# roahmlab/armour

Hardware: AMD Instinct MI355X
Metric: planning iters/s (eval_g+jac) Kinova 7-DOF, 100 timesteps × 20 obstacles (higher is better)
Workload: dtype f64

## Files before the change

armour_amd/csrc/api.hip:

```cpp
#include <algorithm>
#include <cmath>
#include <cstdarg>
#include <chrono>
#include <cstring>
#include <mutex>
#include <new>

#include "../../include/armour_robot_fetch.h"
#include "../../include/armour_robot_kinova.h"
#include "bezier.h"
#include "cacc.h"
#include "common.h"
#include "solver_common.h"

static thread_local char g_err[512] = "";

void armour_set_error(const char* fmt, ...) {
    va_list ap;
    va_start(ap, fmt);
    vsnprintf(g_err, sizeof(g_err), fmt, ap);
    va_end(ap);
}

extern "C" const char* armour_last_error(void) { return g_err; }
// ... 237 lines not shown
    h->d_jac = h->d_g + (size_t)B * h->m;
    const size_t bn = (size_t)B * h->n;
    h->h_q0.assign(q0, q0 + bn); h->h_qd0.assign(qd0, qd0 + bn);
    h->h_qdes.assign(q_des, q_des + bn);
    if (mode == ARMOUR_MODE_ARMTD) { h->h_qdd0.assign(bn, 0.0); h->h_krange.assign(qdd0, qdd0 + bn); }
    else { h->h_qdd0.assign(qdd0, qdd0 + bn); h->h_krange.clear(); }
    std::vector<double> bz((size_t)B * 3 * h->n);
    const double D = mode == ARMOUR_MODE_ARMTD ? 1.0 : h->params.duration;
    for (int b = 0; b < B; b++)
        for (int i = 0; i < h->n; i++) {
            bz[((size_t)b * 3 + 0) * h->n + i] = q0[b * h->n + i];
            bz[((size_t)b * 3 + 1) * h->n + i] = qd0[b * h->n + i] * D;
            bz[((size_t)b * 3 + 2) * h->n + i] = qdd0[b * h->n + i] * D * D;
        }
    HIPCHK(hipMemcpy(h->d_bez, bz.data(), bz.size() * sizeof(double), hipMemcpyHostToDevice));
    return ARMOUR_OK;
}

int armour_refresh_table_stats(ArmourPlanner* h) {
    if (h->stats_fresh) { h->stats_fresh = false; return ARMOUR_OK; }
    const size_t nl = (size_t)h->B * h->J * h->T, nt = (size_t)h->B * h->n * h->T;
    std::vector<int> lc(nl), tc(nt);
    HIPCHK(hipMemcpy(lc.data(), h->d_link_count, nl * sizeof(int), hipMemcpyDeviceToHost));
    HIPCHK(hipMemcpy(tc.data(), h->d_tq_count, nt * sizeof(int), hipMemcpyDeviceToHost));
    long long sl = 0, st = 0;
    int ml = 0, mt = 0;
    for (int v : lc) { sl += v; if (v > ml) ml = v; }
    for (int v : tc) { st += v; if (v > mt) mt = v; }
    h->sum_link = sl; h->sum_torque = st; h->max_link = ml; h->max_torque = mt;
    h->h_plane_skip.assign((size_t)h->B, 0ull);
// ... 221 lines not shown
    if (n < 1 || !q0 || !qd0 || !qdd0 || !k_range || !k || !(duration > 0)) { armour_set_error("bad argument"); return ARMOUR_EINVAL; }
    const double D = duration, s = t / D;
    for (int i = 0; i < n; i++) {
        const double a = qd0[i] * D, b = qdd0[i] * D * D, ka = k_range[i] * k[i];
        if (q) q[i] = bez::q_des(q0[i], a, b, ka, s);
        if (qd) qd[i] = bez::qd_des(q0[i], a, b, ka, s) / D;
        if (qdd) qdd[i] = bez::qdd_des(q0[i], a, b, ka, s) / (D * D);
    }
    return ARMOUR_OK;
}

extern "C" int armour_eval_g_jac_device(ArmourPlanner* h, const double* d_k, double* d_g, double* d_jac, void* stream) {
    NEED_READY(h);
    if (!d_k) { armour_set_error("d_k is null"); return ARMOUR_EINVAL; }
    const P2Tables tb = armour_make_tables(h);
    return armour_p2_launch(tb, h->max_link, h->max_torque, h->h_plane_skip.data(), d_k, d_g, d_jac, stream ? (hipStream_t)stream : h->stream);
}

static int enqueue_steps(ArmourPlanner* h, const double* d_k, int steps, double* d_g, double* d_jac, hipStream_t st) {
    const P2Tables tb = armour_make_tables(h);
    const size_t stride = (size_t)h->B * h->n;
    for (int s = 0; s < steps; s++) {
        int rc = armour_p2_launch(tb, h->max_link, h->max_torque, h->h_plane_skip.data(), d_k + (size_t)s * stride, d_g, d_jac, st);
        if (rc != ARMOUR_OK) return rc;
    }
    return ARMOUR_OK;
}

static int steps_graph(ArmourPlanner* h, const double* d_k, int steps, double* d_g, double* d_jac, hipGraphExec_t* out) {
    h->graph_clock++;
    for (auto& g : h->step_graphs)
        if (g.d_k == d_k && g.steps == steps && g.d_g == d_g && g.d_jac == d_jac) { g.last_use = h->graph_clock; *out = g.exec; return ARMOUR_OK; }
    HIPCHK(hipSetDevice(h->device));
    HIPCHK(hipStreamSynchronize(h->stream));
    hipGraph_t graph = nullptr;
    HIPCHK(hipStreamBeginCapture(h->stream, hipStreamCaptureModeThreadLocal));
    const int rc = enqueue_steps(h, d_k, steps, d_g, d_jac, h->stream);
    const hipError_t e = hipStreamEndCapture(h->stream, &graph);
// ... 38 lines not shown
            if (g.d_k == d_k && g.steps == steps && g.d_g == d_g && g.d_jac == d_jac) {
                g.last_use = ++h->graph_clock;
                HIPCHK(hipGraphLaunch(g.exec, st));
                return ARMOUR_OK;
            }
    return enqueue_steps(h, d_k, steps, d_g, d_jac, st);
}

extern "C" int armour_eval_g_jac_device_multi(ArmourPlanner* h, const double* d_k, int32_t points, double* d_g, double* d_jac,
                                              void* stream) {
    NEED_READY(h);
    if (!d_k || points < 0) { armour_set_error("bad argument"); return ARMOUR_EINVAL; }
    if (points == 0) return ARMOUR_OK;
    const P2Tables tb = armour_make_tables(h);
    const long long bn = (long long)h->B * h->n, bm = (long long)h->B * h->m;
    return armour_p2_launch(tb, h->max_link, h->max_torque, h->h_plane_skip.data(), d_k, d_g, d_jac, stream ? (hipStream_t)stream : h->stream,
                            points, bn, bm, bm * h->n);
}

int armour_spin_on_stream(hipStream_t st) {
    for (;;) {
        const hipError_t q = hipStreamQuery(st);
        if (q == hipSuccess) return ARMOUR_OK;
        if (q != hipErrorNotReady) { armour_set_error("hipStreamQuery failed: %s", hipGetErrorString(q)); return ARMOUR_EDEVICE; }
    }
}

extern "C" int armour_eval_g_jac(ArmourPlanner* h, const double* k, double* g, double* jac) {
    NEED_READY(h);
    if (!k) { armour_set_error("k is null"); return ARMOUR_EINVAL; }
    HIPCHK(hipSetDevice(h->device));
    const size_t bn = (size_t)h->B * h->n, bm = (size_t)h->B * h->m;
    const P2Tables tb = armour_make_tables(h);
    const int pinned_mode = h->tune(ARMOUR_OPT_PINNED_MODE);
    const bool all_pinned = in_pinned(k, bn * sizeof(double)) && in_pinned(g, bm * sizeof(double)) && in_pinned(jac, bm * h->n * sizeof(double));
    if (all_pinned && pinned_mode == 1) {
        int rc = armour_p2_launch(tb, h->max_link, h->max_torque, h->h_plane_skip.data(), k, g, jac, h->stream);
        if (rc != ARMOUR_OK) return rc;
        return armour_spin_on_stream(h->stream);
    }
    const double* k_dev = h->d_k;
    if (all_pinned && pinned_mode == 2) k_dev = k;
    else HIPCHK(hipMemcpyAsync(h->d_k, k, bn * sizeof(double), hipMemcpyHostToDevice, h->stream));
    int rc = armour_p2_launch(tb, h->max_link, h->max_torque, h->h_plane_skip.data(), k_dev, g ? h->d_g : nullptr, jac ? h->d_jac : nullptr, h->stream);
    if (rc != ARMOUR_OK) return rc;
    if (g && jac && jac == g + bm) {
        HIPCHK(hipMemcpyAsync(g, h->d_g, bm * (1 + (size_t)h->n) * sizeof(double), hipMemcpyDeviceToHost, h->stream));
        return armour_spin_on_stream(h->stream);
    }
    if (g) HIPCHK(hipMemcpyAsync(g, h->d_g, bm * sizeof(double), hipMemcpyDeviceToHost, h->stream));
    if (jac) HIPCHK(hipMemcpyAsync(jac, h->d_jac, bm * h->n * sizeof(double), hipMemcpyDeviceToHost, h->stream));
    return armour_spin_on_stream(h->stream);
}

extern "C" int armour_check_feasible(ArmourPlanner* h, const double* g, int32_t* feasible) {
    NEED_READY(h);
    const slv::RowRule R = armour_row_rule(h);
    const slv::RowLimits L = armour_row_limits(h);
    for (int b = 0; b < h->B; b++) {
// ... 116 lines not shown
    for (int r = tid; r < m; r += 256) p[0].take(a.rule, r, g[r], lo[r], hi[r]);
    slv::ViolPartial::tree_reduce(sh, p, tid);
    if (tid == 0) a.out[b] = slv::ViolPartial::finish(sh, 0);
}
}

static int eval_violations_device_impl(ArmourPlanner* h, const double* d_k, ArmourViolation* d_out, void* stream, bool allow_cull) {
    NEED_READY(h);
    if (!d_k || !d_out) { armour_set_error("null argument"); return ARMOUR_EINVAL; }
    HIPCHK(hipSetDevice(h->device));
    int rc = armour_upload_bounds(h);
    if (rc != ARMOUR_OK) return rc;
    const hipStream_t st = stream ? (hipStream_t)stream : h->stream;
    if (allow_cull && h->tune(ARMOUR_OPT_CULL_ROWS)) return armour_eval_violations_culled(h, d_k, d_out, st);
    const P2Tables tb = armour_make_tables(h);
    rc = armour_p2_launch(tb, h->max_link, h->max_torque, h->h_plane_skip.data(), d_k, h->d_g, nullptr, st);
    if (rc != ARMOUR_OK) return rc;
    ViolArgs a;
    a.rule = armour_row_rule(h);
    a.g = h->d_g; a.lo = h->d_bounds; a.hi = h->d_bounds + (size_t)h->B * h->m; a.out = d_out;
    hipLaunchKernelGGL(armour_violation_kernel, dim3(h->B), dim3(256), 0, st, a);
    HIPCHK(hipGetLastError());
    return ARMOUR_OK;
}

extern "C" int armour_eval_violations_device(ArmourPlanner* h, const double* d_k, ArmourViolation* d_out, void* stream) {
    return eval_violations_device_impl(h, d_k, d_out, stream, true);
}

extern "C" int armour_eval_violations(ArmourPlanner* h, const double* k, ArmourViolation* out) {
    NEED_READY(h);
// ... 174 lines not shown
```

armour_amd/csrc/common.h:

```cpp
#pragma once

#include <hip/hip_runtime.h>

#include <cstdint>
#include <cstdio>
#include <string>
#include <vector>

#include "../../include/armour_hip.h"
#include "device_mem.h"
#include "row_rules.h"

#define ARMOUR_NPLANES 36
#define ARMOUR_PLANE_COMPONENTS 5

#define ARMOUR_FIRST_LL_PLANE 21
#define ARMOUR_N_LL_PLANES 15
__host__ __device__ inline int armour_row_stride(int Q) { return (Q + 15) & ~15; }
__host__ __device__ inline size_t armour_planes_ab_offset(int Q) { (void)Q; return 0; }
__host__ __device__ inline size_t armour_planes_cd_offset(int Q) { return (size_t)2 * ARMOUR_NPLANES * armour_row_stride(Q); }
__host__ __device__ inline size_t armour_planes_dll_offset(int Q) { return (size_t)4 * ARMOUR_NPLANES * armour_row_stride(Q); }
__host__ __device__ inline size_t armour_planes_d_offset(int Q) { return (size_t)(4 * ARMOUR_NPLANES + 16) * armour_row_stride(Q); }
__host__ __device__ inline size_t armour_planes_per_problem(int Q) { return (size_t)(5 * ARMOUR_NPLANES + 16) * armour_row_stride(Q); }
__host__ __device__ inline size_t armour_plane_index(int Q, int q, int p, int c) {
// ... 87 lines not shown
    double tune_f(int option) const { return tuning[option - ARMOUR_OPT_FIRST_TUNING]; }
    DevBuf<ArmourViolation> d_viol;
    RelLists rel, rel2;
    int rel2_tq_cap = 0;
    DevBuf<unsigned char> d_sweep;
    SolveDeviceWork solve_dev;
    DevBuf<double> d_bounds;
    bool bounds_on_device = false, bounds_on_host = false;
    bool tables_from_host = false;
    std::vector<double> h_gl, h_gu;
    std::vector<double> h_q0, h_qd0, h_qdd0, h_qdes;
    std::vector<double> h_torque_radius;
    DevBuf<double> d_tr_stage;
    std::vector<double> h_link_gens;
    std::vector<unsigned long long> h_plane_skip;
    std::vector<double> h_prune_margin;
    int allocB = 0, allocO = 0;
    DevBuf<int> d_link_count;
    DevBuf<double> d_link_center;
    DevBuf<double> d_link_indep;
    DevBuf<uint32_t> d_link_keys;
    DevBuf<double> d_link_coeff;
    DevBuf<int> d_tq_count;
    DevBuf<double> d_tq_center;
    DevBuf<double> d_tq_indep;
    DevBuf<uint32_t> d_tq_keys;
    DevBuf<double> d_tq_coeff;
    DevBuf<double> d_planes;
    DevBuf<double> d_obs_center;
    int d_from_center = 0;
// ... 12 lines not shown
    bool p1_two_cu_off = false;
    int p1_hint_B = 0, p1_hint_T = 0, p1_hint_O = 0, p1_hint_builds = 0;
    int build_info[4] = {0, 0, 0, 0};
    int max_link = 0, max_torque = 0;
    long long sum_link = 0, sum_torque = 0;
    void* p1 = nullptr;
    struct StepsGraph { const double* d_k; int steps; double* d_g; double* d_jac; hipGraphExec_t exec; unsigned long long last_use; };
    std::vector<StepsGraph> step_graphs;
    unsigned long long graph_clock = 0;
};

void armour_tuning_defaults(double* tuning);
bool armour_trace_p1();
bool armour_trace_solve();

int armour_p2_launch(const P2Tables& tb, int max_link, int max_torque, const unsigned long long* h_skip, const double* d_k, double* d_g, double* d_jac, hipStream_t stream,
                     int steps = 1, long long k_stride = 0, long long g_stride = 0, long long j_stride = 0, bool skip_collision_blocks = false);
int armour_relevance_build(ArmourPlanner* h, bool for_solver);
int armour_eval_violations_culled(ArmourPlanner* h, const double* d_k, ArmourViolation* d_out, hipStream_t st);
int armour_refresh_table_stats(ArmourPlanner* h);
int armour_checked_collision_rows(const ArmourPlanner* h);
slv::RowRule armour_row_rule(const ArmourPlanner* h);
slv::RowLimits armour_row_limits(const ArmourPlanner* h);
#define NEED_READY(h)                                                                        \
    if (!(h)) { armour_set_error("null handle"); return ARMOUR_EINVAL; }                     \
    if (!(h)->ready) { armour_set_error("no problem set: call armour_set_problems first"); return ARMOUR_ESTATE; }
void armour_plan_coeffs(const ArmourPlanner* h, size_t ix, double c[3]);
double* armour_handle_pinned(ArmourPlanner* h, int slot, size_t bytes);
int armour_p2_slice_links_launch(const P2Tables& tb, const double* d_k, double* d_centers, hipStream_t stream);
P2Tables armour_make_tables(const ArmourPlanner* h);
int armour_upload_bounds(ArmourPlanner* h);
// ... 17 lines not shown
```

armour_amd/csrc/p2_eval.hip:

```cpp
#include "p2_tiles.h"

using namespace p2;

namespace {

template <bool WANT_G, bool WANT_J, bool MULTI, bool DFC, bool LL, int PPW, bool EX>
__global__ __launch_bounds__(P2_BLOCK) __attribute__((amdgpu_waves_per_eu(P2_WPE(DFC, MULTI)))) void armour_p2_eval_kernel(P2Tables tb, const double* __restrict__ k_all,
                                                                  double* __restrict__ g_all, double* __restrict__ jac_all,
                                                                  P2Launch lp) {
    extern __shared__ __attribute__((aligned(16))) unsigned char smem_raw[];
    const int b = blockIdx.y, role = blockIdx.x + lp.role0;
    const int n = tb.n, m = tb.m;
    const double* k0 = k_all + (size_t)b * n;
    double* g0 = WANT_G ? g_all + (size_t)b * m : nullptr;
    double* jac0 = WANT_J ? jac_all + (size_t)b * m * n : nullptr;
    const double k_first = ((int)threadIdx.x < n) ? k0[threadIdx.x] : 0.0;
#ifdef P2_ABLATE
    if ((P2_ABLATE & 1) && role < lp.nbc) return;
    if ((P2_ABLATE & 2) && role >= lp.nbc && role < lp.nbc + lp.nbt) return;
    if ((P2_ABLATE & 4) && role >= lp.nbc + lp.nbt) return;
#endif
    if (role < lp.nbc) collision_block<WANT_G, WANT_J, MULTI, DFC, LL, PPW, EX>(tb, lp, b, role, k0, k_first, g0, jac0, smem_raw);
    else if (role < lp.nbc + lp.nbt) torque_block<WANT_G, WANT_J, MULTI, DFC, LL, PPW, EX>(tb, lp, b, role, k0, k_first, g0, jac0, smem_raw);
    else limit_block<WANT_G, WANT_J, MULTI, DFC, LL, PPW, EX>(tb, lp, b, role, k0, k_first, g0, jac0, smem_raw);
// ... 23 lines not shown

bool armour_p2_ex_layout_ok(unsigned long long skip) {
    unsigned long long live = ~skip & ((1ull << ARMOUR_NPLANES) - 1ull);
    if (__builtin_popcountll(live) != 24) return false;
    int pl[24];
    for (int i = 0; i < 24; i++) { pl[i] = __builtin_ctzll(live); live &= live - 1ull; }
    if (pl[11] >= ARMOUR_FIRST_LL_PLANE || pl[12] < ARMOUR_FIRST_LL_PLANE) return false;
    for (int w = 2; w < 4; w++) {
        const int p0 = pl[6 * w];
        if ((p0 - ARMOUR_FIRST_LL_PLANE) & 1) return false;
        for (int i = 1; i < 6; i++) if (pl[6 * w + i] != p0 + i) return false;
    }
    return true;
}

int armour_p2_plan(const P2Tables& tb, int max_link, int max_torque, const unsigned long long* h_skip, int steps, long long k_stride,
                   long long g_stride, long long j_stride, P2Launch* lp_out, size_t* smem_out, bool* dfc_out, bool* six_out, bool* exact_out) {
    P2Launch lp;
    lp.role0 = 0;
    lp.nbc = (tb.Q + P2_ROWS - 1) / P2_ROWS;
    lp.nbt = tb.row0 == 0 ? 0 : (tb.n * tb.T + P2_TQ_ROWS - 1) / P2_TQ_ROWS;
    lp.max_pairs = tb.O > 0 ? (P2_ROWS - 1) / tb.O + 2 : 1;
    lp.strideL = max_link > 0 ? max_link : 1;
    lp.strideT = max_torque > 0 ? max_torque : 1;
    lp.skip_by_value = (tb.B == 1 && h_skip) ? 1 : 0;
    lp.skip0 = lp.skip_by_value ? h_skip[0] : 0ull;
    lp.steps = steps; lp.k_stride = k_stride; lp.g_stride = g_stride; lp.j_stride = j_stride;
    lp.magic_O = div_magic(tb.O > 0 ? tb.O : 1); lp.magic_pp3 = div_magic(3 * lp.strideL);
    if (tb.Q >= (1 << 20)) { armour_set_error("more than 2^20 collision rows per problem"); return ARMOUR_ECAPACITY; }
    if (lp.strideL * 3 > P2_BLOCK * P2_TASK_ROUNDS) { armour_set_error("link PZ with %d monomials exceeds the P2 kernel's %d", lp.strideL, P2_BLOCK * P2_TASK_ROUNDS / 3); return ARMOUR_ECAPACITY; }
    lp.pair_chunk = std::max(1, std::min(std::min(lp.max_pairs, P2_BLOCK / P2_SL), (P2_BLOCK * P2_TASK_ROUNDS) / (lp.strideL * 3)));
    if (lp.strideT > 32 * P2_TQ_ROUNDS) { armour_set_error("torque PZ with %d monomials exceeds the P2 kernel's %d", lp.strideT, 32 * P2_TQ_ROUNDS); return ARMOUR_ECAPACITY; }
    const size_t col = ((size_t)lp.max_pairs * P2_SL + (size_t)lp.pair_chunk * lp.strideL * P2_SL + 4 * 64 * 4 + 64 * ARMOUR_MAX_FACTORS) * sizeof(double) + 4 * 64 * sizeof(int);
    const size_t tq = (size_t)P2_TQ_ROWS * lp.strideT * P2_TQW * sizeof(double);
    const size_t lim = (size_t)2 * ARMOUR_MAX_FACTORS * 8 * sizeof(double);
    const size_t smem = 2 * sizeof(KPow) + std::max(std::max(col, tq), lim);
    if (smem > 64 * 1024) { armour_set_error("P2 kernel needs %zu B of LDS (link/torque monomial counts too large)", smem); return ARMOUR_ECAPACITY; }
    const bool dfc = tb.obs_center != nullptr && tb.ll_shared;
    bool six = h_skip != nullptr;
    for (int b = 0; six && b < tb.B; b++) six = __builtin_popcountll(~h_skip[b] & ((1ull << ARMOUR_NPLANES) - 1ull)) <= 24;
    bool exact = six && tb.ex_allowed && lp.max_pairs <= lp.pair_chunk;
    for (int b = 0; exact && b < tb.B; b++) exact = armour_p2_ex_layout_ok(h_skip[b]);
    *lp_out = lp; *smem_out = smem; *dfc_out = dfc; *six_out = six; *exact_out = exact;
    return ARMOUR_OK;
}

int armour_p2_launch(const P2Tables& tb, int max_link, int max_torque, const unsigned long long* h_skip, const double* d_k, double* d_g, double* d_jac,
                     hipStream_t stream, int steps, long long k_stride, long long g_stride, long long j_stride, bool skip_collision_blocks) {
    if (!d_g && !d_jac) return ARMOUR_OK;
    P2Launch lp;
    size_t smem = 0;
    bool dfc, six, exact;
    const int rc = armour_p2_plan(tb, max_link, max_torque, h_skip, steps, k_stride, g_stride, j_stride, &lp, &smem, &dfc, &six, &exact);
    if (rc != ARMOUR_OK) return rc;
    if (skip_collision_blocks) lp.role0 = lp.nbc;
    dim3 grid(lp.nbc + lp.nbt + 1 - lp.role0, tb.B), block(P2_BLOCK);
#define P2_LAUNCH_M(G, J, M)                                                                                                                      \
    do {                                                                                                                                          \
        if (dfc && exact && !(M)) hipLaunchKernelGGL((armour_p2_eval_kernel<G, J, false, true, true, 6, true>), grid, block, smem, stream, tb, d_k, d_g, d_jac, lp);      \
        else if (dfc && six) hipLaunchKernelGGL((armour_p2_eval_kernel<G, J, M, true, true, 6, false>), grid, block, smem, stream, tb, d_k, d_g, d_jac, lp);                \
        else if (dfc) hipLaunchKernelGGL((armour_p2_eval_kernel<G, J, M, true, true, 9, false>), grid, block, smem, stream, tb, d_k, d_g, d_jac, lp);              \
        else if (tb.ll_shared && exact && !(M)) hipLaunchKernelGGL((armour_p2_eval_kernel<G, J, false, false, true, 6, true>), grid, block, smem, stream, tb, d_k, d_g, d_jac, lp); \
        else if (tb.ll_shared && six) hipLaunchKernelGGL((armour_p2_eval_kernel<G, J, M, false, true, 6, false>), grid, block, smem, stream, tb, d_k, d_g, d_jac, lp); \
        else if (tb.ll_shared) hipLaunchKernelGGL((armour_p2_eval_kernel<G, J, M, false, true, 9, false>), grid, block, smem, stream, tb, d_k, d_g, d_jac, lp); \
        else hipLaunchKernelGGL((armour_p2_eval_kernel<G, J, M, false, false, 9, false>), grid, block, smem, stream, tb, d_k, d_g, d_jac, lp);             \
    } while (0)
#define P2_LAUNCH(G, J)                                                                                                     \
    do {                                                                                                                    \
// ... 19 lines not shown
```

armour_amd/csrc/p2_tiles.h:

```cpp
#pragma once
#include <algorithm>
#include <cstdlib>

#include "bezier.h"
#include "cacc.h"
#include "common.h"

#define P2_BLOCK 256
#define P2_ROWS 64
#define P2_PPW 9
#define P2_TASK_ROUNDS 2
#define P2_TQ_ROWS 8
#define P2_TQ_ROUNDS 4
#define P2_SL (3 * (1 + ARMOUR_MAX_FACTORS))
#define P2_TQW (1 + ARMOUR_MAX_FACTORS)

#define P2_WPE(DFC, MULTI) ((DFC) && !(MULTI) ? 3 : 1)

namespace p2 {


#ifdef P2_TIMELINE
#define P2_STAMP(i) do { unsigned long long t__; asm volatile("s_memrealtime %0\n\ts_waitcnt lgkmcnt(0)" : "=s"(t__) :: "memory"); stamp[i] = t__; } while (0)
#else
// ... 83 lines not shown

typedef double v2d __attribute__((ext_vector_type(2)));

struct P2Launch {
    int nbc, nbt;
    int role0;
    int max_pairs;
    int strideL;
    int strideT;
    int pair_chunk;
    int skip_by_value;
    unsigned long long skip0;
    int steps;
    long long k_stride, g_stride, j_stride;
    unsigned long long magic_O, magic_pp3;
};

struct PassRegs {
    uint32_t tkey[P2_TASK_ROUNDS];
    double tco[P2_TASK_ROUNDS];
    int tcnt[P2_TASK_ROUNDS], tdst[P2_TASK_ROUNDS];
    double rc_cen, rc_ind;
    int rc_cnt;
};

__device__ inline void load_pass(const P2Tables& tb, const P2Launch& lp, int b, int lt_first, int p0, int pc, PassRegs& pr) {
    const int tid = threadIdx.x;
    const int per_pair = lp.strideL * P2_SL, per_pair3 = lp.strideL * 3;
    const int ntask = pc * per_pair3;
#pragma unroll
// ... 73 lines not shown
    int* pneg = reinterpret_cast<int*>(part + 4 * 64 * 4);
    double* stage = part + 4 * 64 * 4 + 4 * 64 / 2;

    const int q_begin = role * P2_ROWS;
    const int q_end = min(Q, q_begin + P2_ROWS);
    const int q = min(q_begin + lane, q_end - 1);
    const size_t Qs = (size_t)armour_row_stride(Q);
    const double* pl0 = tb.planes + (size_t)b * armour_planes_per_problem(Q);
    const v2d* plAB = reinterpret_cast<const v2d*>(pl0) + q;
    const v2d* plCD = reinterpret_cast<const v2d*>(pl0 + armour_planes_cd_offset(Q)) + q;
    const v2d* plLL = reinterpret_cast<const v2d*>(pl0 + armour_planes_dll_offset(Q)) + q;
    const double* plD = pl0 + armour_planes_d_offset(Q) + q;
    const int JT = tb.J * T;
    const int q_lt = fast_div(q, lp.magic_O), q_o = q - q_lt * O;
    const double* pll = tb.planes_ll + (size_t)b * armour_planes_ll_per_problem(JT) + (size_t)q_lt * ARMOUR_LL_RECORD;
    unsigned long long live = ~(lp.skip_by_value ? lp.skip0 : tb.plane_skip[b]) & ((1ull << ARMOUR_NPLANES) - 1ull);
    const bool plane0_live = (live & 1ull) != 0;
    const int na = __popcll(live), base = na >> 2, rem = na & 3;
    const int my_cnt = base + (wv < rem ? 1 : 0), my_start = wv * base + min(wv, rem);
    for (int s = 0; s < my_start; s++) live &= live - 1ull;
    double a0[PPW], a1[PPW], a2[PPW], dd[PPW], dl[PPW];
    const int lt_first = q_begin / O;
    const int npairs = (q_end - 1) / O - lt_first + 1;
    const bool single_pass = npairs <= lp.pair_chunk;
    PassRegs pr;
    if (EX) load_pass_uncond(tb, lp, b, lt_first, npairs, pr);
    v2d raw[EX ? 12 : 1];
    bool ll_wave = false;
    if (EX) {
        static_assert(!EX || PPW == 6, "the EX kernels hold six planes per wave");
        ll_wave = wv >= 2;
        const v2d* ra[12];
        const double* da[6];
        if (ll_wave) {
            const int pll0 = __builtin_ctzll(live) - ARMOUR_FIRST_LL_PLANE;
            const v2d* nrm = reinterpret_cast<const v2d*>(pll + (size_t)pll0 * 3);
#pragma unroll
            for (int j = 0; j < 9; j++) ra[j] = nrm + j;
// ... 261 lines not shown
}

template <bool WANT_G, bool WANT_J, bool MULTI, bool DFC, bool LL, int PPW, bool EX>
__device__ __forceinline__ void limit_block(const P2Tables& tb, const P2Launch& lp, const int b, const int role, const double* __restrict__ k0,
                                   const double k_first, double* __restrict__ g0_in, double* __restrict__ jac0_in, unsigned char* smem_raw) {
    KPow* kp2 = reinterpret_cast<KPow*>(smem_raw);
    double* lds = reinterpret_cast<double*>(smem_raw + 2 * sizeof(KPow));
    const int n = tb.n, T = tb.T, O = tb.O, Q = tb.Q, m = tb.m;
    const int tid = threadIdx.x, lane = tid & 63;
    const int wv = __builtin_amdgcn_readfirstlane(tid >> 6);
    double* g0 = WANT_G ? g0_in : nullptr;
    double* jac0 = WANT_J ? jac0_in : nullptr;
    const int nsteps = MULTI ? lp.steps : 1;
    double k_next = k_first;
    (void)lane; (void)wv; (void)T; (void)O; (void)Q; (void)m; (void)kp2; (void)lds; (void)g0; (void)jac0; (void)nsteps; (void)k_next;
    double* pv = lds;
    const int jv = tid >> 3, piece = tid & 7;
    const double* bz = tb.bez + (size_t)b * 3 * n;
    if (tb.mode == ARMOUR_MODE_ARMTD) {
        for (int s = 0; s < nsteps; s++) {
            const double* k = k0 + (size_t)s * lp.k_stride;
            double* g = WANT_G ? g0 + (size_t)s * lp.g_stride : nullptr;
            double* jac = WANT_J ? jac0 + (size_t)s * lp.j_stride : nullptr;
            if (tid < n) {
                const cacc::Extrema e = cacc::joint_extrema(bz[tid], bz[n + tid], bz[2 * n + tid] * k[tid]);
                const cacc::Cand c4[4] = {e.q_min, e.q_max, e.qd_min, e.qd_max};
                const size_t off = (size_t)tb.row0 + Q;
                for (int r = 0; r < 4; r++) {
                    const size_t row = off + (size_t)r * n + tid;
                    if (WANT_G) g[row] = c4[r].v;
                    if (WANT_J) for (int c = 0; c < n; c++) jac[row * n + c] = (c == tid) ? c4[r].d : 0.0;
                }
            }
        }
        return;
    }
    for (int s = 0; s < nsteps; s++) {
        const double* k = k0 + (size_t)s * lp.k_stride;
        double* g = WANT_G ? g0 + (size_t)s * lp.g_stride : nullptr;
        double* jac = WANT_J ? jac0 + (size_t)s * lp.j_stride : nullptr;
        if (jv < 2 * n && piece < 6) {
            const int i = jv % n;
            const bool vel = jv >= n;
            const double q0 = bz[i], a = bz[n + i], bb = bz[2 * n + i], ka = tb.k_range[i] * k[i];
            double e2, e3, v;
            if (!vel) bez::q_stationary(a, bb, ka, &e2, &e3); else bez::qd_stationary(a, bb, ka, &e2, &e3);
            if (piece < 4) {
                const double tt = piece == 0 ? 0.0 : piece == 1 ? e2 : piece == 2 ? e3 : 1.0;
                v = vel ? bez::qd_des(q0, a, bb, ka, tt) : bez::q_des(q0, a, bb, ka, tt);
            } else {
                const int sg = piece == 4 ? +1 : -1;
                v = vel ? bez::qd_extremum_dk(q0, a, bb, ka, sg) : bez::q_extremum_dk(q0, a, bb, ka, sg);
            }
            pv[jv * 8 + piece] = v;
            if (piece == 1) pv[jv * 8 + 6] = e2;
            if (piece == 2) pv[jv * 8 + 7] = e3;
        }
        __syncthreads();
        if (tid < 2 * n) {
            const int i = tid % n;
            const bool vel = tid >= n;
            const double* v = pv + tid * 8;
            const double v1 = v[0], v2 = v[1], v3 = v[2], v4 = v[3], e2 = v[6], e3 = v[7];
            double mn, mx;
            int mnId, mxId;
            if (v1 < v4) { mn = v1; mnId = 1; mx = v4; mxId = 4; } else { mn = v4; mnId = 4; mx = v1; mxId = 1; }
            if (0 <= e2 && e2 <= 1) { if (v2 < mn) { mn = v2; mnId = 2; } if (mx < v2) { mx = v2; mxId = 2; } }
            if (0 <= e3 && e3 <= 1) { if (v3 < mn) { mn = v3; mnId = 3; } if (mx < v3) { mx = v3; mxId = 3; } }
            const double sc = vel ? tb.k_range[i] / tb.duration : tb.k_range[i];
            const double dmn = (mnId == 1 ? 0.0 : mnId == 2 ? v[4] : mnId == 3 ? v[5] : 1.0) * sc;
            const double dmx = (mxId == 1 ? 0.0 : mxId == 2 ? v[4] : mxId == 3 ? v[5] : 1.0) * sc;
            const size_t off = (size_t)tb.row0 + Q;
            const size_t r_mn = off + (vel ? 2 * n : 0) + i, r_mx = r_mn + n;
            if (WANT_G) { g[r_mn] = vel ? mn / tb.duration : mn; g[r_mx] = vel ? mx / tb.duration : mx; }
            if (WANT_J) {
                for (int c = 0; c < n; c++) {
                    jac[r_mn * n + c] = (c == i) ? dmn : 0.0;
                    jac[r_mx * n + c] = (c == i) ? dmx : 0.0;
                }
            }
        }
        __syncthreads();
    }
}

}
```

armour_amd/csrc/relevance.hip:

```cpp
#include <vector>

#include "p2_sparse.h"

using namespace p2;

namespace {

constexpr double kRelMargin = 1e-9;

struct RelTables {
    P2Tables tb;
    const double* lo; const double* hi;
    unsigned char* rel;
    unsigned char* rel2;
    int* tq_tiles; int* tq_count; int tq_cap;
    int* rows; int* count;
    int* rows_res; int* count_res;
    double* packed; const long long* pack_off;
};

__device__ inline PlaneVals load_plane(const P2Tables& tb, const double* pl0, const double* pll, int Q, int q, int p, bool dfc, double oc0, double oc1, double oc2) {
    PlaneVals v;
    if (tb.ll_shared && p >= ARMOUR_FIRST_LL_PLANE) {
        const double* al = pll + (size_t)(p - ARMOUR_FIRST_LL_PLANE) * 3;
// ... 353 lines not shown
        if (aux_count) HIPCHK(hipMemcpy(aux_count, L.count + B, B * sizeof(int), hipMemcpyDeviceToHost));
    }
    if (pack_off) {
        std::vector<long long> d_off(2 * B);
        HIPCHK(hipMemcpy(d_off.data(), L.pack_off, 2 * B * sizeof(long long), hipMemcpyDeviceToHost));
        for (size_t i = 0; i < 2 * B; i++) pack_off[i] = d_off[i];
    }
    if (packed && total > 0) HIPCHK(hipMemcpy(packed, L.packed, (size_t)total * sizeof(double), hipMemcpyDeviceToHost));
    return ARMOUR_OK;
}

int armour_eval_violations_culled(ArmourPlanner* h, const double* d_k, ArmourViolation* d_out, hipStream_t st) {
    int rc = armour_relevance_build(h, false);
    if (rc != ARMOUR_OK) return rc;
    const P2Tables tb = armour_make_tables(h);
    rc = armour_p2_launch(tb, h->max_link, h->max_torque, h->h_plane_skip.data(), d_k, h->d_g, nullptr, st, 1, 0, 0, 0, true);
    if (rc != ARMOUR_OK) return rc;
    RelTables a;
    a.tb = tb;
    a.lo = h->d_bounds; a.hi = h->d_bounds + (size_t)h->B * h->m;
    a.rel = h->rel.mask; a.rows = h->rel.rows; a.count = h->rel.count; a.rows_res = h->rel.extra; a.count_res = h->rel.count + (size_t)h->B;
    a.packed = h->rel.packed; a.pack_off = h->rel.pack_off;
    if (h->rel.max_count > 0)
        hipLaunchKernelGGL(armour_sparse_collision_g_kernel, dim3((h->rel.max_count + 63) / 64, h->B), dim3(64), 0, st, a, d_k, h->d_g);
    SparseViolArgs v;
    v.rule = armour_row_rule(h);
    v.g = h->d_g; v.lo = a.lo; v.hi = a.hi; v.rows_res = a.rows_res; v.count_res = a.count_res; v.k = d_k; v.out = d_out;
    hipLaunchKernelGGL(armour_sparse_violation_kernel, dim3(h->B), dim3(256), 0, st, v);
    HIPCHK(hipGetLastError());
    return ARMOUR_OK;
}
// ... 1 lines not shown
```

armour_amd/csrc/solver_device.h:

```cpp
#pragma once
#include "common.h"
#include "p2_tiles.h"
#include "p2_sparse.h"
#include "solver_common.h"

struct alignas(128) SolveCtl {
    unsigned go;
    int pad0;
    double x[slv::NV];
};
struct alignas(64) BlockWord {
    unsigned flag;
    int count;
    int bad;
    int pad0;
    long long viol;
};

struct SolveArgs {
    P2Tables tb;
    p2::P2Launch lp;
    int nb, n_tiles;
    int culled;
    p2::SparseList sl;
// ... 17 lines not shown
    long long budget_ticks;
    long long hard_ticks;
    long long* stamps;
};

struct SolvePlan {
    p2::P2Launch lp;
    size_t smem;
    bool six;
    int n_tiles;
    int capacity;
    double ticks_per_ms;
    const void* fn;
};

int armour_p2_plan(const P2Tables& tb, int max_link, int max_torque, const unsigned long long* h_skip, int steps, long long k_stride,
                   long long g_stride, long long j_stride, p2::P2Launch* lp_out, size_t* smem_out, bool* dfc_out, bool* six_out, bool* exact_out);
int armour_solve_device_capacity(const P2Tables& tb, int max_link, int max_torque, const unsigned long long* h_skip, int device, int b_launch, int waves_per_simd, SolvePlan* plan,
                                 int n_tiles_override = 0);
int armour_solver_lists(ArmourPlanner* h, p2::SparseList* sl, const int** tq_tiles, const int** tq_count, int* tq_cap);
int armour_solve_device_launch(const SolveArgs* d_args, int nb, const SolvePlan& plan, int B, hipStream_t stream);

struct QpProbe {
    double x[slv::NV], gradf[slv::NV], Hd[slv::NV];
    int ncand, pad0;
    double d[slv::NV], max_mult;
    int feasible, attempt, qp_iter[4];
};
int armour_qp_probe_lds_rows(int wps);
int armour_qp_probe(int n, const slv::SolveRow* rows, int wps, int lds_rows, QpProbe* io);
```

armour_amd/csrc/solver_device.hip:

```cpp
#include <algorithm>
#include <atomic>
#include <cmath>
#include <cstring>

#include "bezier.h"
#include "cacc.h"
#include "common.h"
#include "p2_tiles.h"
#include "solver_common.h"
#include "solver_device.h"

using namespace p2;
using namespace slv;

namespace {

enum { CMD_EVAL = 1, CMD_DONE = 4 };
enum { ST_AFTER_FIRST = 0, ST_AFTER_TRIAL = 1, ST_AFTER_RELIN = 2, ST_AFTER_VERDICT = 3 };
constexpr double kInf = 1e300;
#define WAVE_LDS_SYNC() do { __builtin_amdgcn_fence(__ATOMIC_SEQ_CST, "wavefront"); __builtin_amdgcn_wave_barrier(); } while (0)

__device__ inline unsigned ld_coh(const unsigned* p) { return __hip_atomic_load(p, __ATOMIC_RELAXED, __HIP_MEMORY_SCOPE_AGENT); }
__device__ inline int ld_coh(const int* p) { return __hip_atomic_load(p, __ATOMIC_RELAXED, __HIP_MEMORY_SCOPE_AGENT); }
__device__ inline long long ld_coh(const long long* p) { return __hip_atomic_load(p, __ATOMIC_RELAXED, __HIP_MEMORY_SCOPE_AGENT); }
// ... 987 lines not shown
    const size_t smem = (size_t)lds_rows * (NV + 1) * sizeof(double);
    HIPCHK(hipFuncSetAttribute(fn, hipFuncAttributeMaxDynamicSharedMemorySize, (int)smem));
    if (wps == 1) hipLaunchKernelGGL(armour_qp_probe_kernel<1>, dim3(1), dim3(P2_BLOCK), smem, st, d_args.p, d_rows.p, d_io.p);
    else hipLaunchKernelGGL(armour_qp_probe_kernel<2>, dim3(1), dim3(P2_BLOCK), smem, st, d_args.p, d_rows.p, d_io.p);
    HIPCHK(hipGetLastError());
    HIPCHK(hipMemcpyAsync(io, d_io, sizeof(QpProbe), hipMemcpyDeviceToHost, st));
    HIPCHK(hipStreamSynchronize(st));
    return ARMOUR_OK;
}

int armour_solve_device_capacity(const P2Tables& tb, int max_link, int max_torque, const unsigned long long* h_skip, int device, int b_launch, int waves_per_simd, SolvePlan* plan,
                                 int n_tiles_override) {
    P2Launch lp;
    size_t smem = 0;
    bool dfc, six, exact;
    int rc = armour_p2_plan(tb, max_link, max_torque, h_skip, 1, 0, 0, 0, &lp, &smem, &dfc, &six, &exact);
    if (rc != ARMOUR_OK) return rc;
    plan->lp = lp; plan->smem = smem; plan->six = six;
    plan->n_tiles = n_tiles_override > 0 ? n_tiles_override : lp.nbt + lp.nbc + 1;
    int coop = 0;
    HIPCHK(hipDeviceGetAttribute(&coop, hipDeviceAttributeCooperativeLaunch, device));
    if (!coop) { plan->capacity = 0; return ARMOUR_OK; }
    hipDeviceProp_t prop;
    HIPCHK(hipGetDeviceProperties(&prop, device));
    const void* fn1 = !tb.ll_shared ? (const void*)armour_solve_kernel<false, 9, 1> : six ? (const void*)armour_solve_kernel<true, 6, 1> : (const void*)armour_solve_kernel<true, 9, 1>;
    const void* fn2 = !tb.ll_shared ? (const void*)armour_solve_kernel<false, 9, 2> : six ? (const void*)armour_solve_kernel<true, 6, 2> : (const void*)armour_solve_kernel<true, 9, 2>;
    const int wps_env = waves_per_simd;
    const size_t smem1 = std::max(smem, kSolveLdsOnePerCu), smem2 = std::max(smem, kSolveLdsTwoPerCu);
    int per_cu = 0;
    {
        static std::atomic<unsigned long long> set1[3], set2[3];
// ... 27 lines not shown
```

Baseline: 160,200.

## Restructure P2 limit block: pass Bezier coeffs by value, stage rows in LDS

The joint-limit block of the P2 kernel is rewritten. For single-problem launches the Bezier coefficients are passed as kernel arguments. k_range, the coefficients and k are staged in LDS, and the next step's k is prefetched. Work is now split across waves by stationary-point value versus derivative, and the g/jac rows are written through LDS so that one thread stores each (row, column) instead of a serial per-thread column loop. Small tweaks make the skip mask a scalar and use magic division for pair indices. This adds launch argument size and LDS use, plus some extra syncs.

```diff
diff --git a/armour_amd/csrc/api.hip b/armour_amd/csrc/api.hip
--- a/armour_amd/csrc/api.hip
+++ b/armour_amd/csrc/api.hip
@@ -275,6 +275,7 @@
             bz[((size_t)b * 3 + 2) * h->n + i] = qdd0[b * h->n + i] * D * D;
         }
     HIPCHK(hipMemcpy(h->d_bez, bz.data(), bz.size() * sizeof(double), hipMemcpyHostToDevice));
+    h->h_bez = std::move(bz);
     return ARMOUR_OK;
 }
 
@@ -526,14 +527,14 @@
     NEED_READY(h);
     if (!d_k) { armour_set_error("d_k is null"); return ARMOUR_EINVAL; }
     const P2Tables tb = armour_make_tables(h);
-    return armour_p2_launch(tb, h->max_link, h->max_torque, h->h_plane_skip.data(), d_k, d_g, d_jac, stream ? (hipStream_t)stream : h->stream);
+    return armour_p2_launch(tb, h->max_link, h->max_torque, h->h_plane_skip.data(), h->h_bez.data(), d_k, d_g, d_jac, stream ? (hipStream_t)stream : h->stream);
 }
 
 static int enqueue_steps(ArmourPlanner* h, const double* d_k, int steps, double* d_g, double* d_jac, hipStream_t st) {
     const P2Tables tb = armour_make_tables(h);
     const size_t stride = (size_t)h->B * h->n;
     for (int s = 0; s < steps; s++) {
-        int rc = armour_p2_launch(tb, h->max_link, h->max_torque, h->h_plane_skip.data(), d_k + (size_t)s * stride, d_g, d_jac, st);
+        int rc = armour_p2_launch(tb, h->max_link, h->max_torque, h->h_plane_skip.data(), h->h_bez.data(), d_k + (size_t)s * stride, d_g, d_jac, st);
         if (rc != ARMOUR_OK) return rc;
     }
     return ARMOUR_OK;
@@ -602,7 +603,7 @@
     if (points == 0) return ARMOUR_OK;
     const P2Tables tb = armour_make_tables(h);
     const long long bn = (long long)h->B * h->n, bm = (long long)h->B * h->m;
-    return armour_p2_launch(tb, h->max_link, h->max_torque, h->h_plane_skip.data(), d_k, d_g, d_jac, stream ? (hipStream_t)stream : h->stream,
+    return armour_p2_launch(tb, h->max_link, h->max_torque, h->h_plane_skip.data(), h->h_bez.data(), d_k, d_g, d_jac, stream ? (hipStream_t)stream : h->stream,
                             points, bn, bm, bm * h->n);
 }
 
@@ -623,14 +624,14 @@
     const int pinned_mode = h->tune(ARMOUR_OPT_PINNED_MODE);
     const bool all_pinned = in_pinned(k, bn * sizeof(double)) && in_pinned(g, bm * sizeof(double)) && in_pinned(jac, bm * h->n * sizeof(double));
     if (all_pinned && pinned_mode == 1) {
-        int rc = armour_p2_launch(tb, h->max_link, h->max_torque, h->h_plane_skip.data(), k, g, jac, h->stream);
+        int rc = armour_p2_launch(tb, h->max_link, h->max_torque, h->h_plane_skip.data(), h->h_bez.data(), k, g, jac, h->stream);
         if (rc != ARMOUR_OK) return rc;
         return armour_spin_on_stream(h->stream);
     }
     const double* k_dev = h->d_k;
     if (all_pinned && pinned_mode == 2) k_dev = k;
     else HIPCHK(hipMemcpyAsync(h->d_k, k, bn * sizeof(double), hipMemcpyHostToDevice, h->stream));
-    int rc = armour_p2_launch(tb, h->max_link, h->max_torque, h->h_plane_skip.data(), k_dev, g ? h->d_g : nullptr, jac ? h->d_jac : nullptr, h->stream);
+    int rc = armour_p2_launch(tb, h->max_link, h->max_torque, h->h_plane_skip.data(), h->h_bez.data(), k_dev, g ? h->d_g : nullptr, jac ? h->d_jac : nullptr, h->stream);
     if (rc != ARMOUR_OK) return rc;
     if (g && jac && jac == g + bm) {
         HIPCHK(hipMemcpyAsync(g, h->d_g, bm * (1 + (size_t)h->n) * sizeof(double), hipMemcpyDeviceToHost, h->stream));
@@ -777,7 +778,7 @@
     const hipStream_t st = stream ? (hipStream_t)stream : h->stream;
     if (allow_cull && h->tune(ARMOUR_OPT_CULL_ROWS)) return armour_eval_violations_culled(h, d_k, d_out, st);
     const P2Tables tb = armour_make_tables(h);
-    rc = armour_p2_launch(tb, h->max_link, h->max_torque, h->h_plane_skip.data(), d_k, h->d_g, nullptr, st);
+    rc = armour_p2_launch(tb, h->max_link, h->max_torque, h->h_plane_skip.data(), h->h_bez.data(), d_k, h->d_g, nullptr, st);
     if (rc != ARMOUR_OK) return rc;
     ViolArgs a;
     a.rule = armour_row_rule(h);
diff --git a/armour_amd/csrc/common.h b/armour_amd/csrc/common.h
--- a/armour_amd/csrc/common.h
+++ b/armour_amd/csrc/common.h
@@ -125,6 +125,7 @@
     DevBuf<double> d_tr_stage;
     std::vector<double> h_link_gens;
     std::vector<unsigned long long> h_plane_skip;
+    std::vector<double> h_bez;
     std::vector<double> h_prune_margin;
     int allocB = 0, allocO = 0;
     DevBuf<int> d_link_count;
@@ -167,7 +168,7 @@
 bool armour_trace_p1();
 bool armour_trace_solve();
 
-int armour_p2_launch(const P2Tables& tb, int max_link, int max_torque, const unsigned long long* h_skip, const double* d_k, double* d_g, double* d_jac, hipStream_t stream,
+int armour_p2_launch(const P2Tables& tb, int max_link, int max_torque, const unsigned long long* h_skip, const double* h_bez, const double* d_k, double* d_g, double* d_jac, hipStream_t stream,
                      int steps = 1, long long k_stride = 0, long long g_stride = 0, long long j_stride = 0, bool skip_collision_blocks = false);
 int armour_relevance_build(ArmourPlanner* h, bool for_solver);
 int armour_eval_violations_culled(ArmourPlanner* h, const double* d_k, ArmourViolation* d_out, hipStream_t st);
diff --git a/armour_amd/csrc/p2_eval.hip b/armour_amd/csrc/p2_eval.hip
--- a/armour_amd/csrc/p2_eval.hip
+++ b/armour_amd/csrc/p2_eval.hip
@@ -61,7 +61,7 @@
     return true;
 }
 
-int armour_p2_plan(const P2Tables& tb, int max_link, int max_torque, const unsigned long long* h_skip, int steps, long long k_stride,
+int armour_p2_plan(const P2Tables& tb, int max_link, int max_torque, const unsigned long long* h_skip, const double* h_bez, int steps, long long k_stride,
                    long long g_stride, long long j_stride, P2Launch* lp_out, size_t* smem_out, bool* dfc_out, bool* six_out, bool* exact_out) {
     P2Launch lp;
     lp.role0 = 0;
@@ -72,6 +72,9 @@
     lp.strideT = max_torque > 0 ? max_torque : 1;
     lp.skip_by_value = (tb.B == 1 && h_skip) ? 1 : 0;
     lp.skip0 = lp.skip_by_value ? h_skip[0] : 0ull;
+    lp.bez_by_value = (tb.B == 1 && h_bez) ? 1 : 0;
+    for (int c = 0; c < 3; c++)
+        for (int i = 0; i < ARMOUR_MAX_FACTORS; i++) lp.bez0[c * ARMOUR_MAX_FACTORS + i] = (lp.bez_by_value && i < tb.n) ? h_bez[c * tb.n + i] : 0.0;
     lp.steps = steps; lp.k_stride = k_stride; lp.g_stride = g_stride; lp.j_stride = j_stride;
     lp.magic_O = div_magic(tb.O > 0 ? tb.O : 1); lp.magic_pp3 = div_magic(3 * lp.strideL);
     if (tb.Q >= (1 << 20)) { armour_set_error("more than 2^20 collision rows per problem"); return ARMOUR_ECAPACITY; }
@@ -80,7 +83,7 @@
     if (lp.strideT > 32 * P2_TQ_ROUNDS) { armour_set_error("torque PZ with %d monomials exceeds the P2 kernel's %d", lp.strideT, 32 * P2_TQ_ROUNDS); return ARMOUR_ECAPACITY; }
     const size_t col = ((size_t)lp.max_pairs * P2_SL + (size_t)lp.pair_chunk * lp.strideL * P2_SL + 4 * 64 * 4 + 64 * ARMOUR_MAX_FACTORS) * sizeof(double) + 4 * 64 * sizeof(int);
     const size_t tq = (size_t)P2_TQ_ROWS * lp.strideT * P2_TQW * sizeof(double);
-    const size_t lim = (size_t)2 * ARMOUR_MAX_FACTORS * 8 * sizeof(double);
+    const size_t lim = (size_t)(2 * ARMOUR_MAX_FACTORS * 8 + 2 * ARMOUR_MAX_FACTORS + 3 * 4 * ARMOUR_MAX_FACTORS) * sizeof(double);
     const size_t smem = 2 * sizeof(KPow) + std::max(std::max(col, tq), lim);
     if (smem > 64 * 1024) { armour_set_error("P2 kernel needs %zu B of LDS (link/torque monomial counts too large)", smem); return ARMOUR_ECAPACITY; }
     const bool dfc = tb.obs_center != nullptr && tb.ll_shared;
@@ -92,13 +95,13 @@
     return ARMOUR_OK;
 }
 
-int armour_p2_launch(const P2Tables& tb, int max_link, int max_torque, const unsigned long long* h_skip, const double* d_k, double* d_g, double* d_jac,
+int armour_p2_launch(const P2Tables& tb, int max_link, int max_torque, const unsigned long long* h_skip, const double* h_bez, const double* d_k, double* d_g, double* d_jac,
                      hipStream_t stream, int steps, long long k_stride, long long g_stride, long long j_stride, bool skip_collision_blocks) {
     if (!d_g && !d_jac) return ARMOUR_OK;
     P2Launch lp;
     size_t smem = 0;
     bool dfc, six, exact;
-    const int rc = armour_p2_plan(tb, max_link, max_torque, h_skip, steps, k_stride, g_stride, j_stride, &lp, &smem, &dfc, &six, &exact);
+    const int rc = armour_p2_plan(tb, max_link, max_torque, h_skip, h_bez, steps, k_stride, g_stride, j_stride, &lp, &smem, &dfc, &six, &exact);
     if (rc != ARMOUR_OK) return rc;
     if (skip_collision_blocks) lp.role0 = lp.nbc;
     dim3 grid(lp.nbc + lp.nbt + 1 - lp.role0, tb.B), block(P2_BLOCK);
diff --git a/armour_amd/csrc/p2_tiles.h b/armour_amd/csrc/p2_tiles.h
--- a/armour_amd/csrc/p2_tiles.h
+++ b/armour_amd/csrc/p2_tiles.h
@@ -121,6 +121,8 @@
     int steps;
     long long k_stride, g_stride, j_stride;
     unsigned long long magic_O, magic_pp3;
+    int bez_by_value;
+    double bez0[3 * ARMOUR_MAX_FACTORS];
 };
 
 struct PassRegs {
@@ -224,14 +226,16 @@
     const int JT = tb.J * T;
     const int q_lt = fast_div(q, lp.magic_O), q_o = q - q_lt * O;
     const double* pll = tb.planes_ll + (size_t)b * armour_planes_ll_per_problem(JT) + (size_t)q_lt * ARMOUR_LL_RECORD;
-    unsigned long long live = ~(lp.skip_by_value ? lp.skip0 : tb.plane_skip[b]) & ((1ull << ARMOUR_NPLANES) - 1ull);
+    unsigned long long skip0 = lp.skip0;
+    asm volatile("" : "+s"(skip0));
+    unsigned long long live = ~(lp.skip_by_value ? skip0 : tb.plane_skip[b]) & ((1ull << ARMOUR_NPLANES) - 1ull);
     const bool plane0_live = (live & 1ull) != 0;
     const int na = __popcll(live), base = na >> 2, rem = na & 3;
     const int my_cnt = base + (wv < rem ? 1 : 0), my_start = wv * base + min(wv, rem);
     for (int s = 0; s < my_start; s++) live &= live - 1ull;
     double a0[PPW], a1[PPW], a2[PPW], dd[PPW], dl[PPW];
-    const int lt_first = q_begin / O;
-    const int npairs = (q_end - 1) / O - lt_first + 1;
+    const int lt_first = fast_div(q_begin, lp.magic_O);
+    const int npairs = fast_div(q_end - 1, lp.magic_O) - lt_first + 1;
     const bool single_pass = npairs <= lp.pair_chunk;
     PassRegs pr;
     if (EX) load_pass_uncond(tb, lp, b, lt_first, npairs, pr);
@@ -523,74 +527,106 @@
     const int nsteps = MULTI ? lp.steps : 1;
     double k_next = k_first;
     (void)lane; (void)wv; (void)T; (void)O; (void)Q; (void)m; (void)kp2; (void)lds; (void)g0; (void)jac0; (void)nsteps; (void)k_next;
+    static_assert(P2_BLOCK >= 4 * ARMOUR_MAX_FACTORS * 8 && ARMOUR_MAX_FACTORS <= 8, "the store pass holds one (row, column) per thread: 4n rows x 8 columns");
     double* pv = lds;
-    const int jv = tid >> 3, piece = tid & 7;
+    double* kb = pv + 2 * ARMOUR_MAX_FACTORS * 8;
+    double* sg = kb + 2 * ARMOUR_MAX_FACTORS;
+    double* sd = sg + 4 * ARMOUR_MAX_FACTORS;
+    double* cs = sd + 4 * ARMOUR_MAX_FACTORS;
     const double* bz = tb.bez + (size_t)b * 3 * n;
-    if (tb.mode == ARMOUR_MODE_ARMTD) {
-        for (int s = 0; s < nsteps; s++) {
-            const double* k = k0 + (size_t)s * lp.k_stride;
-            double* g = WANT_G ? g0 + (size_t)s * lp.g_stride : nullptr;
-            double* jac = WANT_J ? jac0 + (size_t)s * lp.j_stride : nullptr;
-            if (tid < n) {
-                const cacc::Extrema e = cacc::joint_extrema(bz[tid], bz[n + tid], bz[2 * n + tid] * k[tid]);
-                const cacc::Cand c4[4] = {e.q_min, e.q_max, e.qd_min, e.qd_max};
-                const size_t off = (size_t)tb.row0 + Q;
-                for (int r = 0; r < 4; r++) {
-                    const size_t row = off + (size_t)r * n + tid;
-                    if (WANT_G) g[row] = c4[r].v;
-                    if (WANT_J) for (int c = 0; c < n; c++) jac[row * n + c] = (c == tid) ? c4[r].d : 0.0;
+    const bool armtd = tb.mode == ARMOUR_MODE_ARMTD;
+    const size_t off = (size_t)tb.row0 + Q;
+    const bool by_value = lp.bez_by_value != 0;
+    if (lane == 0) {
+        if (wv == 0) {
+#pragma unroll
+            for (int j = 0; j < ARMOUR_MAX_FACTORS; j++) cs[j] = tb.k_range[j];
+        } else if (by_value) {
+#pragma unroll
+            for (int c = 1; c < 4; c++) {
+                if (wv == c) {
+#pragma unroll
+                    for (int j = 0; j < ARMOUR_MAX_FACTORS; j++) cs[c * ARMOUR_MAX_FACTORS + j] = lp.bez0[(c - 1) * ARMOUR_MAX_FACTORS + j];
                 }
             }
         }
-        return;
-    }
+    }
+    if (!by_value && tid < 3 * n) {
+        const int c = tid >= 2 * n ? 2 : tid >= n ? 1 : 0;
+        cs[(1 + c) * ARMOUR_MAX_FACTORS + tid - c * n] = bz[tid];
+    }
+    if (tid < n) kb[tid] = k_first;
+    __syncthreads();
     for (int s = 0; s < nsteps; s++) {
-        const double* k = k0 + (size_t)s * lp.k_stride;
+        const double k_cur = k_next;
+        if (tid < n && s + 1 < nsteps) k_next = k0[(size_t)(s + 1) * lp.k_stride + tid];
         double* g = WANT_G ? g0 + (size_t)s * lp.g_stride : nullptr;
         double* jac = WANT_J ? jac0 + (size_t)s * lp.j_stride : nullptr;
-        if (jv < 2 * n && piece < 6) {
-            const int i = jv % n;
-            const bool vel = jv >= n;
-            const double q0 = bz[i], a = bz[n + i], bb = bz[2 * n + i], ka = tb.k_range[i] * k[i];
-            double e2, e3, v;
-            if (!vel) bez::q_stationary(a, bb, ka, &e2, &e3); else bez::qd_stationary(a, bb, ka, &e2, &e3);
-            if (piece < 4) {
-                const double tt = piece == 0 ? 0.0 : piece == 1 ? e2 : piece == 2 ? e3 : 1.0;
-                v = vel ? bez::qd_des(q0, a, bb, ka, tt) : bez::q_des(q0, a, bb, ka, tt);
-            } else {
-                const int sg = piece == 4 ? +1 : -1;
-                v = vel ? bez::qd_extremum_dk(q0, a, bb, ka, sg) : bez::q_extremum_dk(q0, a, bb, ka, sg);
-            }
-            pv[jv * 8 + piece] = v;
-            if (piece == 1) pv[jv * 8 + 6] = e2;
-            if (piece == 2) pv[jv * 8 + 7] = e3;
+        if (armtd) {
+            if (tid < n) {
+                const double c0 = cs[ARMOUR_MAX_FACTORS + tid], c1 = cs[2 * ARMOUR_MAX_FACTORS + tid], c2 = cs[3 * ARMOUR_MAX_FACTORS + tid];
+                const cacc::Extrema e = cacc::joint_extrema(c0, c1, c2 * k_cur);
+                const cacc::Cand c4[4] = {e.q_min, e.q_max, e.qd_min, e.qd_max};
+#pragma unroll
+                for (int r = 0; r < 4; r++) { sg[r * n + tid] = c4[r].v; sd[r * n + tid] = c4[r].d; }
+            }
+        } else {
+            const bool is_dk = wv >= 2, vel = (wv & 1) != 0;
+            const int i = is_dk ? lane >> 1 : lane >> 2;
+            if (i < n) {
+                const int jv = vel ? n + i : i;
+                const double q0 = cs[ARMOUR_MAX_FACTORS + i], a = cs[2 * ARMOUR_MAX_FACTORS + i], bb = cs[3 * ARMOUR_MAX_FACTORS + i];
+                const double ka = cs[i] * kb[(s & 1) * ARMOUR_MAX_FACTORS + i];
+                double v;
+                if (!is_dk) {
+                    const int piece = lane & 3;
+                    double e2, e3;
+                    if (!vel) bez::q_stationary(a, bb, ka, &e2, &e3); else bez::qd_stationary(a, bb, ka, &e2, &e3);
+                    const double tt = piece == 0 ? 0.0 : piece == 1 ? e2 : piece == 2 ? e3 : 1.0;
+                    if (!vel) v = bez::q_des(q0, a, bb, ka, tt); else v = bez::qd_des(q0, a, bb, ka, tt);
+                    pv[jv * 8 + piece] = v;
+                    if (piece == 1) pv[jv * 8 + 6] = e2;
+                    if (piece == 2) pv[jv * 8 + 7] = e3;
+                } else {
+                    const int sgn = (lane & 1) ? -1 : +1;
+                    if (!vel) v = bez::q_extremum_dk(q0, a, bb, ka, sgn); else v = bez::qd_extremum_dk(q0, a, bb, ka, sgn);
+                    pv[jv * 8 + 4 + (lane & 1)] = v;
+                }
+            }
+            __syncthreads();
+            if (tid < n && s + 1 < nsteps) kb[((s + 1) & 1) * ARMOUR_MAX_FACTORS + tid] = k_next;
+            if (tid < 2 * n) {
+                const bool velr = tid >= n;
+                const int ir = velr ? tid - n : tid;
+                const double* v = pv + tid * 8;
+                const double v1 = v[0], v2 = v[1], v3 = v[2], v4 = v[3], e2 = v[6], e3 = v[7];
+                double mn, mx;
+                int mnId, mxId;
+                if (v1 < v4) { mn = v1; mnId = 1; mx = v4; mxId = 4; } else { mn = v4; mnId = 4; mx = v1; mxId = 1; }
+                if (0 <= e2 && e2 <= 1) { if (v2 < mn) { mn = v2; mnId = 2; } if (mx < v2) { mx = v2; mxId = 2; } }
+                if (0 <= e3 && e3 <= 1) { if (v3 < mn) { mn = v3; mnId = 3; } if (mx < v3) { mx = v3; mxId = 3; } }
+                const double kr = cs[ir];
+                const double sc = velr ? kr / tb.duration : kr;
+                const double dmn = (mnId == 1 ? 0.0 : mnId == 2 ? v[4] : mnId == 3 ? v[5] : 1.0) * sc;
+                const double dmx = (mxId == 1 ? 0.0 : mxId == 2 ? v[4] : mxId == 3 ? v[5] : 1.0) * sc;
+                const int r_mn = (velr ? 2 * n : 0) + ir, r_mx = r_mn + n;
+                sg[r_mn] = velr ? mn / tb.duration : mn; sg[r_mx] = velr ? mx / tb.duration : mx;
+                sd[r_mn] = dmn; sd[r_mx] = dmx;
+            }
         }
         __syncthreads();
-        if (tid < 2 * n) {
-            const int i = tid % n;
-            const bool vel = tid >= n;
-            const double* v = pv + tid * 8;
-            const double v1 = v[0], v2 = v[1], v3 = v[2], v4 = v[3], e2 = v[6], e3 = v[7];
-            double mn, mx;
-            int mnId, mxId;
-            if (v1 < v4) { mn = v1; mnId = 1; mx = v4; mxId = 4; } else { mn = v4; mnId = 4; mx = v1; mxId = 1; }
-            if (0 <= e2 && e2 <= 1) { if (v2 < mn) { mn = v2; mnId = 2; } if (mx < v2) { mx = v2; mxId = 2; } }
-            if (0 <= e3 && e3 <= 1) { if (v3 < mn) { mn = v3; mnId = 3; } if (mx < v3) { mx = v3; mxId = 3; } }
-            const double sc = vel ? tb.k_range[i] / tb.duration : tb.k_range[i];
-            const double dmn = (mnId == 1 ? 0.0 : mnId == 2 ? v[4] : mnId == 3 ? v[5] : 1.0) * sc;
-            const double dmx = (mxId == 1 ? 0.0 : mxId == 2 ? v[4] : mxId == 3 ? v[5] : 1.0) * sc;
-            const size_t off = (size_t)tb.row0 + Q;
-            const size_t r_mn = off + (vel ? 2 * n : 0) + i, r_mx = r_mn + n;
-            if (WANT_G) { g[r_mn] = vel ? mn / tb.duration : mn; g[r_mx] = vel ? mx / tb.duration : mx; }
-            if (WANT_J) {
-                for (int c = 0; c < n; c++) {
-                    jac[r_mn * n + c] = (c == i) ? dmn : 0.0;
-                    jac[r_mx * n + c] = (c == i) ? dmx : 0.0;
-                }
-            }
-        }
-        __syncthreads();
-    }
-}
-
-}
+        if (WANT_G && tid < 4 * n) g[off + tid] = sg[tid];
+        if (WANT_J) {
+            const int r = tid >> 3, c = tid & 7;
+            if (r < 4 * n && c < n) {
+                int ir = r;
+                if (ir >= 2 * n) ir -= 2 * n;
+                if (ir >= n) ir -= n;
+                jac[(off + r) * n + c] = (c == ir) ? sd[r] : 0.0;
+            }
+        }
+        if (MULTI && armtd) __syncthreads();
+    }
+}
+
+}
diff --git a/armour_amd/csrc/relevance.hip b/armour_amd/csrc/relevance.hip
--- a/armour_amd/csrc/relevance.hip
+++ b/armour_amd/csrc/relevance.hip
@@ -391,7 +391,7 @@
     int rc = armour_relevance_build(h, false);
     if (rc != ARMOUR_OK) return rc;
     const P2Tables tb = armour_make_tables(h);
-    rc = armour_p2_launch(tb, h->max_link, h->max_torque, h->h_plane_skip.data(), d_k, h->d_g, nullptr, st, 1, 0, 0, 0, true);
+    rc = armour_p2_launch(tb, h->max_link, h->max_torque, h->h_plane_skip.data(), h->h_bez.data(), d_k, h->d_g, nullptr, st, 1, 0, 0, 0, true);
     if (rc != ARMOUR_OK) return rc;
     RelTables a;
     a.tb = tb;
diff --git a/armour_amd/csrc/solver_device.h b/armour_amd/csrc/solver_device.h
--- a/armour_amd/csrc/solver_device.h
+++ b/armour_amd/csrc/solver_device.h
@@ -55,7 +55,7 @@
     const void* fn;
 };
 
-int armour_p2_plan(const P2Tables& tb, int max_link, int max_torque, const unsigned long long* h_skip, int steps, long long k_stride,
+int armour_p2_plan(const P2Tables& tb, int max_link, int max_torque, const unsigned long long* h_skip, const double* h_bez, int steps, long long k_stride,
                    long long g_stride, long long j_stride, p2::P2Launch* lp_out, size_t* smem_out, bool* dfc_out, bool* six_out, bool* exact_out);
 int armour_solve_device_capacity(const P2Tables& tb, int max_link, int max_torque, const unsigned long long* h_skip, int device, int b_launch, int waves_per_simd, SolvePlan* plan,
                                  int n_tiles_override = 0);
diff --git a/armour_amd/csrc/solver_device.hip b/armour_amd/csrc/solver_device.hip
--- a/armour_amd/csrc/solver_device.hip
+++ b/armour_amd/csrc/solver_device.hip
@@ -1025,7 +1025,7 @@
     P2Launch lp;
     size_t smem = 0;
     bool dfc, six, exact;
-    int rc = armour_p2_plan(tb, max_link, max_torque, h_skip, 1, 0, 0, 0, &lp, &smem, &dfc, &six, &exact);
+    int rc = armour_p2_plan(tb, max_link, max_torque, h_skip, nullptr, 1, 0, 0, 0, &lp, &smem, &dfc, &six, &exact);
     if (rc != ARMOUR_OK) return rc;
     plan->lp = lp; plan->smem = smem; plan->six = six;
     plan->n_tiles = n_tiles_override > 0 ? n_tiles_override : lp.nbt + lp.nbc + 1;
```

New measurement: 170,700, median of 6. 6.6% higher.
